# iclavera/learning_to_adapt

Hardware: AMD Instinct MI355X
Metric: controller-steps/sec (n_cand=2000, H=30, ens=5) (higher is better)
Workload: dtype f32

## Files before the change

### learning_to_adapt_amd/csrc/l2a_mfma.h

```cpp
#pragma once

#include <type_traits>

#include "l2a_kernels.h"

#ifndef L2A_XEARLY
#define L2A_XEARLY 1
#endif

#ifndef L2A_NW
#define L2A_NW 4
#endif

typedef unsigned int u32x4 __attribute__((ext_vector_type(4)));
__device__ __forceinline__ __amdgpu_buffer_rsrc_t l2a_rsrc(const void* base, long long bytes) {
    return __builtin_amdgcn_make_buffer_rsrc(const_cast<void*>(base), 0, (int)bytes, 0x00020000);
}
__device__ __forceinline__ f32x4 l2a_ldw(__amdgpu_buffer_rsrc_t rs, int voff, int soff) {
    return __builtin_bit_cast(f32x4, __builtin_amdgcn_raw_buffer_load_b128(rs, voff, soff, 0));
}

template <bool GACT>
__device__ __forceinline__ f32x4 l2a_actv(f32x4 v, int kind, float floor) {
    if (GACT) return l2a_act4(v, kind);
    v.x = l2a_max_nan(v.x, floor); v.y = l2a_max_nan(v.y, floor);
    v.z = l2a_max_nan(v.z, floor); v.w = l2a_max_nan(v.w, floor);
    return v;
}

__device__ __forceinline__ float l2a_sum_xor16(float x) {
    const unsigned int u = __float_as_uint(x);
    const auto r = __builtin_amdgcn_permlane16_swap(u, u, false, false);
    return __uint_as_float(r[0]) + __uint_as_float(r[1]);
}
__device__ __forceinline__ float l2a_sum_xor32(float x) {
    const unsigned int u = __float_as_uint(x);
    const auto r = __builtin_amdgcn_permlane32_swap(u, u, false, false);
    return __uint_as_float(r[0]) + __uint_as_float(r[1]);
}

#define L2A_MFMA4(a, b, c) __builtin_amdgcn_mfma_f32_4x4x1f32((a), (b), (c), 0, 0, 0)

#define L2A_OPAQUE(v) asm volatile("" : "+v"(v))

#ifndef L2A_TIMELINE
#define L2A_TS(slot)
#else
#define L2A_TS(slot)                                                                        \
    if (p.dbg && pairid == 0 && e < 8 && grp < 2) {                                         \
        unsigned long long ts_;                                                             \
        asm volatile("s_memtime %0\n\ts_waitcnt lgkmcnt(0)" : "=s"(ts_) : : "memory");       \
        if (lane == 0) p.dbg[(((long long)(grp * p.h + t) * 8 + e) * 8 + wave) * 16 + (slot)] = ts_; \
    }
#endif

#define L2A_STAGE_MFMA(CA, CB)                                                             \
    _Pragma("unroll") for (int ii = 0; ii < 4; ++ii)                                       \
        _Pragma("unroll") for (int nt = 0; nt < NT; ++nt)                                  \
            _Pragma("unroll") for (int tt = TW - 1; tt >= 0; --tt)    \
                acc[nt][tt] = L2A_MFMA(CA[tt][ii], CB[nt][ii], acc[nt][tt]);

#define L2A_STAGE(CA, CB, FA, FB, SOFF, IMM, GF)                                           \
    {                                                                                      \
        _Pragma("unroll") for (int tt = 0; tt < TW; ++tt)                                  \
            FA[tt] = l2a_ldw(rs, voff[tt] + (IMM), (SOFF));                                \
        _Pragma("unroll") for (int nt = 0; nt < NT; ++nt)                                  \
            FB[nt] = hin[(nt * HT + (GF)) * 64 + lane];                                    \
        L2A_STAGE_MFMA(CA, CB)                                                             \
         \
        __builtin_amdgcn_sched_group_barrier(0x100, NT, 0);                                \
        _Pragma("unroll") for (int tt = 0; tt < TW; ++tt) {                                \
            __builtin_amdgcn_sched_group_barrier(0x008, 4 * NT, 0);                        \
            __builtin_amdgcn_sched_group_barrier(0x020, 1, 0);                             \
        }                                                                                  \
        __builtin_amdgcn_sched_barrier(0);                                                 \
    }

#define L2A_PFT_MAX 6
#define L2A_PFT(TW_, OT_) ((OT_) <= 2 ? ((TW_) < L2A_PFT_MAX ? (TW_) : L2A_PFT_MAX) : ((TW_) < 2 ? (TW_) : 2))

template <int NT, int TW, int TPW, int OT, bool LAST>
__device__ __forceinline__ void l2a_hidden_gemm(__amdgpu_buffer_rsrc_t rs, __amdgpu_buffer_rsrc_t rsn,
                                                const int (&voff)[TPW], const int (&voffn)[TPW], int twn,
                                                int tile0, const f32x4* hin,
                                                f32x4 (&aA)[TPW], f32x4 (&aB)[TPW],
                                                f32x4 (&pfO)[TPW][OT], f32x4 (&acc)[NT][TPW], int lane,
                                                const float* bias_lds, f32x4 (&bias)[TPW], const int (&olane)[OT]) {
    constexpr int HT = L2A_NW * TPW;
    static_assert(HT % 4 == 0, "the k-group pipeline is unrolled by 4");
    f32x4 aC[TW], aD[TW], bA[NT], bB[NT], bC[NT], bD[NT];
#pragma unroll
    for (int nt = 0; nt < NT; ++nt) {
        bA[nt] = hin[(nt * HT + 0) * 64 + lane];
        bB[nt] = hin[(nt * HT + 1) * 64 + lane];
#pragma unroll
        for (int tt = 0; tt < TW; ++tt) acc[nt][tt] = (f32x4){0.f, 0.f, 0.f, 0.f};
    }
#pragma unroll
    for (int nt = 0; nt < NT; ++nt) { L2A_OPAQUE(bA[nt]); L2A_OPAQUE(bB[nt]); }
    __builtin_amdgcn_sched_barrier(0);

#pragma unroll 1
    for (int g = 0; g < HT - 4; g += 4) {
        const int soff = (g + 2) * 1024;
        L2A_STAGE(aA, bA, aC, bC, soff, 0, g + 2)
        L2A_STAGE(aB, bB, aD, bD, soff, 1024, g + 3)
        L2A_STAGE(aC, bC, aA, bA, soff, 2048, g + 4)
        L2A_STAGE(aD, bD, aB, bB, soff, 3072, g + 5)
    }
    L2A_STAGE(aA, bA, aC, bC, (HT - 2) * 1024, 0, HT - 2)
    L2A_STAGE(aB, bB, aD, bD, (HT - 2) * 1024, 1024, HT - 1)
    {
        if (LAST) {
#pragma unroll
            for (int tt = 0; tt < L2A_PFT(TW, OT); ++tt)
#pragma unroll
                for (int c = 0; c < OT; ++c)
                    if (((tt * OT + c) & 1) == 0)
                        pfO[tt][c] = l2a_ldw(rsn, olane[c] + (tile0 + tt) * 1024, c * HT * 1024);
        } else {
#pragma unroll
            for (int tt = 0; tt < TPW; ++tt)
                if (tt < twn) aA[tt] = l2a_ldw(rsn, voffn[tt], 0);
        }
        L2A_STAGE_MFMA(aC, bC)
        __builtin_amdgcn_sched_barrier(0);
    }
    {
#pragma unroll
        for (int tt = 0; tt < TW; ++tt) bias[tt] = *reinterpret_cast<const f32x4*>(bias_lds + 16 * tt);
        if (LAST) {
#pragma unroll
            for (int tt = 0; tt < L2A_PFT(TW, OT); ++tt)
#pragma unroll
                for (int c = 0; c < OT; ++c)
                    if (((tt * OT + c) & 1) == 1)
                        pfO[tt][c] = l2a_ldw(rsn, olane[c] + (tile0 + tt) * 1024, c * HT * 1024);
        } else {
#pragma unroll
            for (int tt = 0; tt < TPW; ++tt)
                if (tt < twn) aB[tt] = l2a_ldw(rsn, voffn[tt] + 1024, 0);
        }
        L2A_STAGE_MFMA(aD, bD)
        __builtin_amdgcn_sched_barrier(0);
    }
}

template <int NT, int TW, int TPW, int OT, int NPF, bool O4, class PF>
__device__ __forceinline__ void l2a_out_phase(const f32x4 (&hreg)[NT][TPW], f32x4 (&pfO)[TPW][OT],
                                              __amdgpu_buffer_rsrc_t rs_out, int tile0, PF prefetch,
                                              f32x4* pbuf, int chunk0, int lane, const int (&olane)[OT]) {
    constexpr int HT = L2A_NW * TPW;
    constexpr int CS = TPW / 2;
    constexpr int NCH = TW / CS;
    f32x4 a[TW][OT];
#pragma unroll
    for (int tt = 0; tt < TW; ++tt)
#pragma unroll
        for (int c = 0; c < OT; ++c)
            a[tt][c] = (tt < L2A_PFT(TW, OT)) ? pfO[tt][c]
                                              : l2a_ldw(rs_out, olane[c] + (tile0 + tt) * 1024, c * HT * 1024);
    prefetch();
    f32x4 acc[NCH][NT][OT];
#pragma unroll
    for (int ch = 0; ch < NCH; ++ch)
#pragma unroll
        for (int nt = 0; nt < NT; ++nt)
#pragma unroll
            for (int c = 0; c < OT; ++c) acc[ch][nt][c] = (f32x4){0.f, 0.f, 0.f, 0.f};
#pragma unroll
    for (int t2 = 0; t2 < CS; ++t2)
#pragma unroll
        for (int ii = 0; ii < 4; ++ii)
#pragma unroll
            for (int ch = 0; ch < NCH; ++ch)
#pragma unroll
                for (int nt = 0; nt < NT; ++nt)
#pragma unroll
                    for (int c = 0; c < OT; ++c)
                        acc[ch][nt][c] = (O4 && c == OT - 1)
                            ? L2A_MFMA4(a[ch * CS + t2][c][ii], hreg[nt][ch * CS + t2][ii], acc[ch][nt][c])
                            : L2A_MFMA(a[ch * CS + t2][c][ii], hreg[nt][ch * CS + t2][ii], acc[ch][nt][c]);
    {
        constexpr int NLATE = (TW - L2A_PFT(TW, OT)) * OT;
        constexpr int NMFMA = TW * 4 * NT * OT;
#pragma unroll
        for (int i = 0; i < NLATE; ++i) {
            __builtin_amdgcn_sched_group_barrier(0x020, 1, 0);
            __builtin_amdgcn_sched_group_barrier(0x008, 2, 0);
        }
        constexpr int PER = (NMFMA - 2 * NLATE) / NPF > 0 ? (NMFMA - 2 * NLATE) / NPF : 1;
#pragma unroll
        for (int i = 0; i < NPF; ++i) {
            __builtin_amdgcn_sched_group_barrier(0x008, PER, 0);
            __builtin_amdgcn_sched_group_barrier(0x020, 1, 0);
        }
    }
#pragma unroll
    for (int nt = 0; nt < NT; ++nt)
#pragma unroll
        for (int c = 0; c < OT; ++c)
            pbuf[((chunk0 * NT + nt) * OT + c) * 64 + lane] = (NCH == 2) ? acc[0][nt][c] + acc[NCH - 1][nt][c] : acc[0][nt][c];
}

template <int NT, int TPW, int OT, int KG0, bool GACT, int K0L = 4, bool N1 = false, bool O4 = false, bool FAN = false, bool WHOLE = false>
__global__ void __launch_bounds__(64 * L2A_NW) l2a_rollout_mfma_k(const L2AKParams p) {
    static_assert(!(FAN && WHOLE), "an instance is general, member fan or whole-tiles-only");
    constexpr bool NOHALF = FAN || WHOLE;
    constexpr int HT = L2A_NW * TPW;
    constexpr int TH = TPW / 2;
    static_assert(TPW % 2 == 0, "half members split a wave's tiles in two");
    constexpr int CST_BOUT = 32 * KG0 + 32 * OT;
    constexpr int CST_BHID = CST_BOUT + 16 * OT;
    constexpr int PS = L2A_NW * NT * OT * 64;
    const int NRM_SET = p.cst_set;
    const int LB = p.lb;
    extern __shared__ __attribute__((aligned(16))) char l2a_smem[];
    f32x4* buf0 = reinterpret_cast<f32x4*>(l2a_smem);
    f32x4* buf1 = buf0 + p.sa_elems;
    f32x4* pbase = buf0 + (LB > 1 ? LB : 2) * p.sa_elems;
    float* nrm = reinterpret_cast<float*>(buf0 + p.cst_off);

    const int tid = threadIdx.x;
    const int lane = tid & 63;
    const int wave = __builtin_amdgcn_readfirstlane(tid >> 6);
    const int jc = lane & 15;
    const int qq = lane >> 4;
    const int c0 = wave * TPW;
    int olane[OT];
#pragma unroll
    for (int c = 0; c < OT; ++c) olane[c] = ((O4 && c == OT - 1) ? ((lane & 48) | (lane & 3)) : lane) * 16;

    const int tail = p.split_from >= 0;
    const int in_tail = tail && (int)blockIdx.x >= p.split_from;
    const int split = FAN ? 3 : WHOLE ? 0 : (tail ? (in_tail ? p.split : 0) : p.split);
    const int n_tiles = p.m * p.tiles_per_env;
    const int n_pairs = tail ? n_tiles - p.split_from : n_tiles;
    int bid, grp, lpair, pairid;
    if (!tail && p.pl_units > 0) {
        const int hx = (int)blockIdx.x & 7, idx = (int)blockIdx.x >> 3;
        const int xcd = hx;
        const int f = p.pl_f, wide = p.pl_r * (f + 1);
        int u, k, xu;
        if (xcd < wide) { u = xcd / (f + 1); k = xcd - u * (f + 1); xu = f + 1; }
        else { const int y = xcd - wide; u = y / f; k = y - u * f; u += p.pl_r; xu = f; }
        const int su = (p.pl_w + xu - 1) / xu;
        const int j = k * su + idx;
        if (idx >= su || j >= p.pl_w) return;
        if (p.mode == L2A_MODE_PER_BLOCK) {
            grp = split ? j / p.tiles_per_env : 0;
            lpair = u * p.tiles_per_env + (j - grp * p.tiles_per_env);
        } else {
            grp = u;
            lpair = j;
        }
        bid = grp * n_pairs + lpair;
        pairid = lpair;
    } else if (!tail) {
        bid = l2a_logical_wg(blockIdx.x, gridDim.x);
        grp = split ? (bid / n_pairs) : 0;
        lpair = bid - grp * n_pairs;
        pairid = lpair;
    } else if (!in_tail) {
        bid = l2a_logical_wg(blockIdx.x, p.split_from);
        grp = 0; lpair = 0; pairid = bid;
    } else {
        bid = (int)blockIdx.x - p.split_from;
        grp = bid & 1; lpair = bid >> 1;
        pairid = p.split_from + lpair;
    }
#if defined(L2A_TIMELINE) || defined(L2A_WGREC)
    unsigned long long wg_t0_, wg_r0_;
    asm volatile("s_memtime %0\n\ts_memrealtime %1\n\ts_waitcnt lgkmcnt(0)" : "=s"(wg_t0_), "=s"(wg_r0_) : : "memory");
#endif
    const int env = pairid / p.tiles_per_env;
    const int tb = pairid - env * p.tiles_per_env;
    const int R = p.m * p.n;
    const int obs_dim = p.obs_dim, act_dim = p.act_dim;
    const int n_hidden = N1 ? 1 : p.n_hidden;

    int cand[NT], row[NT];
    bool valid[NT];
#pragma unroll
    for (int nt = 0; nt < NT; ++nt) {
        cand[nt] = p.c_lo + tb * (16 * NT) + nt * 16 + jc;
        valid[nt] = cand[nt] < p.c_hi;
        row[nt] = env * p.n + (valid[nt] ? cand[nt] : p.c_hi - 1);
    }

    const bool per_block = (p.mode == L2A_MODE_PER_BLOCK);
    const int e_loop = (p.mode == L2A_MODE_MEAN) ? p.n_sets : 1;
    const int e_half = (e_loop + 1) >> 1;
    const int e_shared = (!NOHALF && split == 2) ? e_half - 1 : -1;
    const int n_full = FAN ? 1 : (!split ? e_loop : (grp == 0 ? e_half - (split == 2 ? 1 : 0) : e_loop - e_half));
    const int n_seq = FAN ? 1 : n_full + (split == 2 ? 1 : 0);
    const int full0 = FAN ? grp : ((split && grp == 1) ? e_half : 0);
    auto seq = [&](int i) { return (i < n_full) ? full0 + i : e_shared; };
    auto set_base = [&](int e) { return p.wblk + (long long)(per_block ? env : e) * p.set_stride; };

    f32x4* xlds = reinterpret_cast<f32x4*>(nrm + p.n_cst * NRM_SET);
    for (int i = tid; i < n_seq * NRM_SET; i += 64 * L2A_NW) {
        const int s = i / NRM_SET;
        const int o = i - s * NRM_SET;
        const float* src = set_base(seq(s));
        float v;
        if (o < CST_BOUT) v = src[p.nm_off + o];
        else if (o < CST_BHID) v = src[p.pk_bout + (o - CST_BOUT)];
        else {
            const int l = (o - CST_BHID) / (16 * HT);
            v = src[p.raw_b[l] + (o - CST_BHID - l * 16 * HT)];
        }
        nrm[i] = v;
    }

    f32x4 st[NT][OT];
#pragma unroll
    for (int nt = 0; nt < NT; ++nt) {
        const float* orow = p.obs0 + (p.obs_per_row ? (long long)row[nt] : (long long)env) * obs_dim;
#pragma unroll
        for (int c = 0; c < OT; ++c)
#pragma unroll
            for (int ii = 0; ii < 4; ++ii) {
                const int dim = 16 * c + 4 * qq + ii;
                const float v = orow[dim < obs_dim ? dim : obs_dim - 1];
                st[nt][c][ii] = (dim < obs_dim) ? v : 0.0f;
            }
    }
    __syncthreads();

    const int ga0 = obs_dim >> 4;
    f32x4 av_next[NT][2];
    int aoff[NT][2][4];
#pragma unroll
    for (int nt = 0; nt < NT; ++nt)
#pragma unroll
        for (int s = 0; s < 2; ++s)
#pragma unroll
            for (int ii = 0; ii < 4; ++ii) {
                const int ka = 16 * (ga0 + s) + 4 * qq + ii - obs_dim;
                const bool in = (ka >= 0) && (ka < act_dim);
                aoff[nt][s][ii] = in ? (row[nt] * act_dim + ka) * 4 : 0x7ffffff0;
            }
    const long long a_step = (long long)R * act_dim;
    auto load_actions = [&](int t, f32x4 (&dst)[NT][2]) {
        const __amdgpu_buffer_rsrc_t ars = l2a_rsrc(p.actions + (long long)t * a_step, a_step * 4);
#pragma unroll
        for (int nt = 0; nt < NT; ++nt)
#pragma unroll
            for (int s = 0; s < 2; ++s)
#pragma unroll
                for (int ii = 0; ii < 4; ++ii)
                    dst[nt][s][ii] = __builtin_bit_cast(float, __builtin_amdgcn_raw_buffer_load_b32(ars, aoff[nt][s][ii], 0, 0));
    };
    f32x4 av[NT][2];
    float asq[NT];
    auto take_actions = [&](int t_fetch) {
#pragma unroll
        for (int nt = 0; nt < NT; ++nt) {
            av[nt][0] = av_next[nt][0];
            av[nt][1] = av_next[nt][1];
            float s = 0.0f;
#pragma unroll
            for (int ii = 0; ii < 4; ++ii) {
                s = fmaf(av[nt][0][ii], av[nt][0][ii], s);
                s = fmaf(av[nt][1][ii], av[nt][1][ii], s);
            }
            asq[nt] = s;
        }
        load_actions((t_fetch < p.h) ? t_fetch : p.h - 1, av_next);
    };
    load_actions(0, av_next);
    take_actions(1);

    float ret[NT];
#pragma unroll
    for (int nt = 0; nt < NT; ++nt) ret[nt] = p.ret_in ? p.ret_in[(long long)env * p.n + (valid[nt] ? cand[nt] : p.c_hi - 1)] : 0.0f;

    f32x4* hcur = buf0;
    f32x4* hoth = buf1;
    const float e_count = (float)e_loop;
    const float e_inv = 1.0f / e_count;
    double disc_pow = p.disc0;
    unsigned int spin_left = p.spin_limit;
    const unsigned int xtag0 = p.xtag;
    const __amdgpu_buffer_rsrc_t xrs = l2a_rsrc(p.xbuf, FAN ? (long long)n_pairs * e_loop * 2 * (NT * OT * 2 * 64 * 16)
                                                        : split ? (long long)n_pairs * 8 * (NT * OT * 2 * 64 * 16) : 16);

    constexpr int KG0P = (FAN && KG0 <= 2) ? KG0 : 1;
    f32x4 pfL0[KG0P][TPW];
    f32x4 pfA[TPW], pfB[TPW];
    f32x4 pfO[TPW][OT];
    int voff[TPW], voffh[TPW], voff0[TPW];
    const int tile0h = grp * (HT / 2) + wave * TH;
#pragma unroll
    for (int tt = 0; tt < TPW; ++tt) {
        voff[tt] = lane * 16 + (c0 + tt) * HT * 1024;
        voffh[tt] = lane * 16 + (tile0h + (tt < TH ? tt : 0)) * HT * 1024;
        voff0[tt] = lane * 16 + (c0 + tt) * KG0 * 1024;
    }
    const long long w0_bytes = (long long)HT * KG0 * 1024, wm_bytes = (long long)HT * HT * 1024,
                    wo_bytes = (long long)OT * HT * 1024;
    {
        const __amdgpu_buffer_rsrc_t r0 = l2a_rsrc(set_base(seq(0)) + p.pk_w0, w0_bytes);
#pragma unroll
        for (int g = 0; g < KG0P; ++g)
#pragma unroll
            for (int tt = 0; tt < TPW; ++tt) pfL0[g][tt] = l2a_ldw(r0, voff0[tt] + g * 1024, 0);
    }

    for (int t = 0; t < p.h; ++t) {
        f32x4 dsum[NT][OT], dgrp[NT][OT], qsh[NT][OT];
#pragma unroll
        for (int nt = 0; nt < NT; ++nt)
#pragma unroll
            for (int c = 0; c < OT; ++c) {
                dsum[nt][c] = (f32x4){0.f, 0.f, 0.f, 0.f};
                dgrp[nt][c] = (f32x4){0.f, 0.f, 0.f, 0.f};
                qsh[nt][c] = (f32x4){0.f, 0.f, 0.f, 0.f};
            }

        const unsigned int xtag = xtag0 + (unsigned int)(t + 1);
        constexpr int XREG = NT * OT * 2 * 64 * 16;
        auto xbase = [&](int g, int region) { return (((lpair * 2 + g) * 2 + (t & 1)) * 2 + region) * XREG + lane * 16; };
        auto xput = [&](int region, const f32x4 (&v)[NT][OT]) {
#pragma unroll
            for (int nt = 0; nt < NT; ++nt)
#pragma unroll
                for (int c = 0; c < OT; ++c)
#pragma unroll
                    for (int hh = 0; hh < 2; ++hh) {
                        u32x4 g;
                        g.x = xtag; g.y = __float_as_uint(v[nt][c][2 * hh]);
                        g.z = xtag; g.w = __float_as_uint(v[nt][c][2 * hh + 1]);
                        __builtin_amdgcn_raw_buffer_store_b128(g, xrs, xbase(grp, region) + ((nt * OT + c) * 2 + hh) * 1024, 0, L2A_SC1);
                    }
        };
        auto xget = [&](int region, f32x4 (&v)[NT][OT]) {
            bool ok = true;
#pragma unroll
            for (int nt = 0; nt < NT; ++nt)
#pragma unroll
                for (int c = 0; c < OT; ++c)
#pragma unroll
                    for (int hh = 0; hh < 2; ++hh) {
                        const u32x4 g = __builtin_amdgcn_raw_buffer_load_b128(
                            xrs, xbase(grp ^ 1, region) + ((nt * OT + c) * 2 + hh) * 1024, 0, L2A_SC1);
                        v[nt][c][2 * hh] = __uint_as_float(g.y);
                        v[nt][c][2 * hh + 1] = __uint_as_float(g.w);
                        ok = ok && (g.x == xtag) && (g.z == xtag);
                    }
            return ok;
        };

        bool xearly = false;
        u32x4 sw[2][NT][OT][2];
        for (int b0 = 0; b0 < n_seq; b0 += LB) {
            const int nb = (n_seq - b0 < LB) ? n_seq - b0 : LB;
            f32x4 hreg[NT][TPW];

            auto layer0 = [&](int j, auto last_tag) {
                constexpr bool last_l0 = decltype(last_tag)::value;
                const int i = b0 + j;
                const int e = seq(i);
                const float* wb = set_base(e);
                const float* nr = nrm + i * NRM_SET;
                const __amdgpu_buffer_rsrc_t rs_out = l2a_rsrc(wb + p.pk_wout, wo_bytes);
                L2A_TS(0)
                const __amdgpu_buffer_rsrc_t r0 = l2a_rsrc(wb + p.pk_w0, w0_bytes);
                f32x4 a[KG0][TPW];
#pragma unroll
                for (int g = 0; g < KG0; ++g)
#pragma unroll
                    for (int tt = 0; tt < TPW; ++tt)
                        a[g][tt] = (g < KG0P) ? pfL0[g < KG0P ? g : 0][tt] : l2a_ldw(r0, voff0[tt] + g * 1024, 0);
                L2A_TS(8)
                constexpr bool XPRE = (KG0 <= 2);
                auto norm_in = [&](int g, const f32x4& mu, const f32x4& iv, f32x4 (&x)[NT]) {
#pragma unroll
                    for (int nt = 0; nt < NT; ++nt) {
                        f32x4 sv = (f32x4){0.f, 0.f, 0.f, 0.f};
                        if (g < OT) sv = st[nt][g < OT ? g : 0];
                        f32x4 aa = (f32x4){0.f, 0.f, 0.f, 0.f};
                        if (g == ga0) aa = av[nt][0];
                        if (g == ga0 + 1) aa = av[nt][1];
#pragma unroll
                        for (int ii = 0; ii < 4; ++ii) x[nt][ii] = ((sv[ii] + aa[ii]) - mu[ii]) * iv[ii];
                    }
                };
                f32x4 xin[XPRE ? KG0 : 1][NT];
                if (XPRE) {
                    f32x4 mu[KG0], iv[KG0];
#pragma unroll
                    for (int g = 0; g < KG0; ++g) {
                        mu[g] = *reinterpret_cast<const f32x4*>(nr + 16 * g + 4 * qq);
                        iv[g] = *reinterpret_cast<const f32x4*>(nr + 16 * KG0 + 16 * g + 4 * qq);
                    }
                    __builtin_amdgcn_sched_barrier(0);
#pragma unroll
                    for (int g = 0; g < KG0; ++g) norm_in(g, mu[g], iv[g], xin[XPRE ? g : 0]);
                }
                f32x4 bias0[TPW];
#pragma unroll
                for (int tt = 0; tt < TPW; ++tt)
                    bias0[tt] = *reinterpret_cast<const f32x4*>(nr + CST_BHID + 16 * (c0 + tt) + 4 * qq);
                f32x4 acc[NT][TPW];
                auto l0_mfma = [&](auto npf_tag) {
                    constexpr int NPF = decltype(npf_tag)::value;
#pragma unroll
                    for (int nt = 0; nt < NT; ++nt)
#pragma unroll
                        for (int tt = 0; tt < TPW; ++tt) acc[nt][tt] = (f32x4){0.f, 0.f, 0.f, 0.f};
#pragma unroll
                    for (int g = 0; g < KG0; ++g) {
                        f32x4 xg[NT];
                        if (XPRE) {
#pragma unroll
                            for (int nt = 0; nt < NT; ++nt) xg[nt] = xin[XPRE ? g : 0][nt];
                        } else {
                            const f32x4 mu = *reinterpret_cast<const f32x4*>(nr + 16 * g + 4 * qq);
                            const f32x4 iv = *reinterpret_cast<const f32x4*>(nr + 16 * KG0 + 16 * g + 4 * qq);
                            norm_in(g, mu, iv, xg);
                        }
#pragma unroll
                        for (int ii = 0; ii < 4; ++ii) {
                            if (g == KG0 - 1 && ii >= K0L) continue;
#pragma unroll
                            for (int nt = 0; nt < NT; ++nt)
#pragma unroll
                                for (int tt = 0; tt < TPW; ++tt)
                                    acc[nt][tt] = L2A_MFMA(a[g][tt][ii], xg[nt][ii], acc[nt][tt]);
                        }
                    }
                    constexpr int NM = ((KG0 - 1) * 4 + K0L) * NT * TPW;
                    constexpr int PER = NM / (NPF > 0 ? NPF : 1) > 0 ? NM / (NPF > 0 ? NPF : 1) : 1;
                    __builtin_amdgcn_sched_group_barrier(0x020, (KG0 - KG0P) * TPW, 0);
#pragma unroll
                    for (int k = 0; k < NPF; ++k) {
                        __builtin_amdgcn_sched_group_barrier(0x008, PER, 0);
                        __builtin_amdgcn_sched_group_barrier(0x020, 1, 0);
                    }
                };
                if (N1) {
#pragma unroll
                    for (int tt = 0; tt < L2A_PFT(TPW, OT); ++tt)
#pragma unroll
                        for (int c = 0; c < OT; ++c)
                            pfO[tt][c] = l2a_ldw(rs_out, olane[c] + (c0 + tt) * 1024, c * HT * 1024);
                    l0_mfma(std::integral_constant<int, L2A_PFT(TPW, OT) * OT>{});
                } else if (!last_l0) {
                    const __amdgpu_buffer_rsrc_t r0n = l2a_rsrc(set_base(seq(i + 1)) + p.pk_w0, w0_bytes);
#pragma unroll
                    for (int g = 0; g < KG0P; ++g)
#pragma unroll
                        for (int tt = 0; tt < TPW; ++tt) pfL0[g][tt] = l2a_ldw(r0n, voff0[tt] + g * 1024, 0);
                    l0_mfma(std::integral_constant<int, KG0P * TPW>{});
                } else {
                    const int e0 = seq(b0);
                    const __amdgpu_buffer_rsrc_t rs1 = l2a_rsrc(set_base(e0) + p.pk_wmid, wm_bytes);
                    const bool next_half = !NOHALF && (e0 == e_shared) && n_hidden == 2;
                    if (next_half) {
#pragma unroll
                        for (int tt = 0; tt < TH; ++tt) {
                            pfA[tt] = l2a_ldw(rs1, voffh[tt], 0);
                            pfB[tt] = l2a_ldw(rs1, voffh[tt] + 1024, 0);
                        }
                        l0_mfma(std::integral_constant<int, 2 * TH>{});
                    } else {
#pragma unroll
                        for (int tt = 0; tt < TPW; ++tt) {
                            pfA[tt] = l2a_ldw(rs1, voff[tt], 0);
                            pfB[tt] = l2a_ldw(rs1, voff[tt] + 1024, 0);
                        }
                        l0_mfma(std::integral_constant<int, 2 * TPW>{});
                    }
                }
                L2A_TS(9)
#pragma unroll
                for (int tt = 0; tt < TPW; ++tt) {
#pragma unroll
                    for (int nt = 0; nt < NT; ++nt)
                        hreg[nt][tt] = l2a_actv<GACT>(acc[nt][tt] + bias0[tt], p.hidden_act, p.hid_floor);
                }
                L2A_TS(10)
                if (!N1) {
                    f32x4* hdst = (LB > 1) ? buf0 + j * p.sa_elems : hcur;
#pragma unroll
                    for (int tt = 0; tt < TPW; ++tt)
#pragma unroll
                        for (int nt = 0; nt < NT; ++nt) hdst[(nt * HT + c0 + tt) * 64 + lane] = hreg[nt][tt];
                }
                L2A_TS(1)
            };

            auto member = [&](int j, auto last_tag) {
                constexpr bool last_set = decltype(last_tag)::value;
                const int i = b0 + j;
                const int e = seq(i);
                const bool is_half = !NOHALF && last_set && (e == e_shared);
                const float* wb = set_base(e);
                const float* nr = nrm + i * NRM_SET;
                const __amdgpu_buffer_rsrc_t rs_out = l2a_rsrc(wb + p.pk_wout, wo_bytes);
                f32x4* pb = (LB > 1) ? pbase + j * PS : hoth;
                L2A_TS(2)
                if (!N1) {
                    f32x4 acc[NT][TPW], bias[TPW];
                    for (int l = 1; last_set && l < n_hidden - 1; ++l) {
                        const float* wl = wb + p.pk_wmid + (long long)(l - 1) * p.pk_wmid_stride;
                        const bool next_half = is_half && (l == n_hidden - 2);
                        l2a_hidden_gemm<NT, TPW, TPW, OT, false>(l2a_rsrc(wl, wm_bytes), l2a_rsrc(wl + p.pk_wmid_stride, wm_bytes),
                                                                 voff, next_half ? voffh : voff, next_half ? TH : TPW, 0,
                                                                 hcur, pfA, pfB, pfO, acc, lane,
                                                                 nr + CST_BHID + l * (16 * HT) + 16 * c0 + 4 * qq, bias, olane);
#pragma unroll
                        for (int tt = 0; tt < TPW; ++tt) {
#pragma unroll
                            for (int nt = 0; nt < NT; ++nt)
                                hoth[(nt * HT + c0 + tt) * 64 + lane] = l2a_actv<GACT>(acc[nt][tt] + bias[tt], p.hidden_act, p.hid_floor);
                        }
                        __syncthreads();
                        f32x4* tmp = hcur; hcur = hoth; hoth = tmp;
                    }
                    if (LB == 1) pb = hoth;
                    L2A_TS(15)
                    const f32x4* hin = (LB > 1) ? buf0 + j * p.sa_elems : hcur;
                    const __amdgpu_buffer_rsrc_t rs_last =
                        l2a_rsrc(wb + p.pk_wmid + (long long)(n_hidden - 2) * p.pk_wmid_stride, wm_bytes);
                    const float* bl = nr + CST_BHID + (n_hidden - 1) * (16 * HT);
                    if (!is_half) {
                        l2a_hidden_gemm<NT, TPW, TPW, OT, true>(rs_last, rs_out, voff, voff, TPW, c0, hin, pfA, pfB, pfO,
                                                                acc, lane, bl + 16 * c0 + 4 * qq, bias, olane);
#pragma unroll
                        for (int tt = 0; tt < TPW; ++tt) {
#pragma unroll
                            for (int nt = 0; nt < NT; ++nt)
                                hreg[nt][tt] = l2a_actv<GACT>(acc[nt][tt] + bias[tt], p.hidden_act, p.hid_floor);
                        }
                    } else {
                        l2a_hidden_gemm<NT, TH, TPW, OT, true>(rs_last, rs_out, voffh, voffh, TH, tile0h, hin, pfA, pfB,
                                                               pfO, acc, lane, bl + 16 * tile0h + 4 * qq, bias, olane);
#pragma unroll
                        for (int tt = 0; tt < TH; ++tt) {
#pragma unroll
                            for (int nt = 0; nt < NT; ++nt)
                                hreg[nt][tt] = l2a_actv<GACT>(acc[nt][tt] + bias[tt], p.hidden_act, p.hid_floor);
                        }
                    }
                }
                L2A_TS(3)
                if (last_set) {
                    const __amdgpu_buffer_rsrc_t r0n = l2a_rsrc(set_base(seq((i + 1 < n_seq) ? i + 1 : 0)) + p.pk_w0, w0_bytes);
                    auto pf_l0 = [&]() {
#pragma unroll
                        for (int g = 0; g < KG0P; ++g)
#pragma unroll
                            for (int tt = 0; tt < TPW; ++tt) pfL0[g][tt] = l2a_ldw(r0n, voff0[tt] + g * 1024, 0);
                    };
                    if (is_half) l2a_out_phase<NT, TH, TPW, OT, KG0P * TPW, O4>(hreg, pfO, rs_out, tile0h, pf_l0, pb, wave, lane, olane);
                    else l2a_out_phase<NT, TPW, TPW, OT, KG0P * TPW, O4>(hreg, pfO, rs_out, c0, pf_l0, pb, wave, lane, olane);
                } else {
                    const int en = seq(i + 1);
                    const __amdgpu_buffer_rsrc_t rsn = l2a_rsrc(set_base(en) + p.pk_wmid, wm_bytes);
                    if (!NOHALF && en == e_shared) {
                        l2a_out_phase<NT, TPW, TPW, OT, 2 * TH, O4>(hreg, pfO, rs_out, c0, [&]() {
#pragma unroll
                            for (int tt = 0; tt < TH; ++tt) {
                                pfA[tt] = l2a_ldw(rsn, voffh[tt], 0);
                                pfB[tt] = l2a_ldw(rsn, voffh[tt] + 1024, 0);
                            }
                        }, pb, wave, lane, olane);
                    } else {
                        l2a_out_phase<NT, TPW, TPW, OT, 2 * TPW, O4>(hreg, pfO, rs_out, c0, [&]() {
#pragma unroll
                            for (int tt = 0; tt < TPW; ++tt) {
                                pfA[tt] = l2a_ldw(rsn, voff[tt], 0);
                                pfB[tt] = l2a_ldw(rsn, voff[tt] + 1024, 0);
                            }
                        }, pb, wave, lane, olane);
                    }
                }
                L2A_TS(4)
            };
            for (int j = 0; j + 1 < nb; ++j) layer0(j, std::false_type{});
            layer0(nb - 1, std::true_type{});
            if (!N1) __syncthreads();
            for (int j = 0; j + 1 < nb; ++j) member(j, std::false_type{});
            member(nb - 1, std::true_type{});

            __syncthreads();
            constexpr bool XE_OK = L2A_XEARLY && !NOHALF && NT == 1 && OT <= 2 && KG0 <= 2;
            const bool xe = XE_OK && split == 2 && nb >= 2 && b0 + nb == n_seq;
            for (int jj = 0; jj < nb; ++jj) {
                const int j = (xe && wave == 0) ? (jj == 0 ? nb - 1 : jj - 1) : jj;
                const int i = b0 + j;
                const int e = seq(i);
                const bool is_half = !NOHALF && (e == e_shared);
                const float* nr = nrm + i * NRM_SET;
                const f32x4* pb = (LB > 1) ? pbase + j * PS : hoth;
                L2A_TS(5)
                if (e == e_half && !split) {
#pragma unroll
                    for (int nt = 0; nt < NT; ++nt)
#pragma unroll
                        for (int c = 0; c < OT; ++c) {
                            dsum[nt][c] = dgrp[nt][c];
                            dgrp[nt][c] = (f32x4){0.f, 0.f, 0.f, 0.f};
                        }
                }
#pragma unroll
                for (int c = 0; c < OT; ++c) {
                    f32x4 part[L2A_NW][NT];
#pragma unroll
                    for (int ch = 0; ch < L2A_NW; ++ch)
#pragma unroll
                        for (int nt = 0; nt < NT; ++nt) part[ch][nt] = pb[((ch * NT + nt) * OT + c) * 64 + lane];
                    const f32x4 bias = *reinterpret_cast<const f32x4*>(nr + CST_BOUT + 16 * c + 4 * qq);
                    const f32x4 omu = *reinterpret_cast<const f32x4*>(nr + 32 * KG0 + 16 * c + 4 * qq);
                    const f32x4 osd = *reinterpret_cast<const f32x4*>(nr + 32 * KG0 + 16 * OT + 16 * c + 4 * qq);
                    __builtin_amdgcn_sched_barrier(0);
#pragma unroll
                    for (int nt = 0; nt < NT; ++nt) {
                        static_assert(L2A_NW == 4, "the canonical tree below is written out for four waves");
                        f32x4 s = (part[0][nt] + part[1][nt]) + (part[2][nt] + part[3][nt]);
                        if (is_half) {
                            qsh[nt][c] = s;
                        } else {
                            if (O4 && c == OT - 1) {
#pragma unroll
                                for (int ii = 0; ii < 4; ++ii) s[ii] = l2a_sum_xor32(l2a_sum_xor16(s[ii]));
                            }
                            s = l2a_actv<GACT>(s + bias, p.output_act, p.out_floor);
                            if (FAN) dgrp[nt][c] = s * osd + omu;
                            else dgrp[nt][c] += s * osd + omu;
                        }
                    }
                }
                if (!NOHALF && split == 2 && i == n_full - 1 && wave == (XE_OK ? 1 : 0)) xput(0, dgrp);
                if (xe && wave == 0 && jj == 0) xput(1, qsh);
                if (xe && wave == 3 && jj == nb - 1) {
#pragma unroll
                    for (int r = 0; r < 2; ++r)
#pragma unroll
                        for (int nt = 0; nt < NT; ++nt)
#pragma unroll
                            for (int c = 0; c < OT; ++c)
#pragma unroll
                                for (int hh = 0; hh < 2; ++hh)
                                    sw[r][nt][c][hh] = (r == 1 || e_loop > 1)
                                        ? __builtin_amdgcn_raw_buffer_load_b128(xrs, xbase(grp ^ 1, r) + ((nt * OT + c) * 2 + hh) * 1024, 0, L2A_SC1)
                                        : (u32x4){xtag, 0u, xtag, 0u};
                }
                L2A_TS(6)
            }
            if (xe) xearly = true;
            if (N1) { f32x4* tmp = hcur; hcur = hoth; hoth = tmp; }
        }

        { const int e = 7; L2A_TS(9) }
        float asq_t[NT];
#pragma unroll
        for (int nt = 0; nt < NT; ++nt) asq_t[nt] = asq[nt];
        if (FAN) {
            constexpr int XREGF = NT * OT * 2 * 64 * 16;
            auto fbase = [&](int g) { return ((lpair * e_loop + g) * 2 + (t & 1)) * XREGF + lane * 16; };
            if (wave == 0) {
#pragma unroll
                for (int nt = 0; nt < NT; ++nt)
#pragma unroll
                    for (int c = 0; c < OT; ++c) {
#pragma unroll
                        for (int hh = 0; hh < 2; ++hh) {
                            u32x4 g;
                            g.x = xtag; g.y = __float_as_uint(dgrp[nt][c][2 * hh]);
                            g.z = xtag; g.w = __float_as_uint(dgrp[nt][c][2 * hh + 1]);
                            __builtin_amdgcn_raw_buffer_store_b128(g, xrs, fbase(grp) + ((nt * OT + c) * 2 + hh) * 1024, 0, L2A_SC1);
                        }
                        xlds[((grp * NT + nt) * OT + c) * 64 + lane] = dgrp[nt][c];
                    }
            }
            { const int e = 7; L2A_TS(11) }
            take_actions(t + 2);
            for (int k = wave; k < e_loop - 1; k += L2A_NW) {
                int g2 = grp + 1 + k;
                if (g2 >= e_loop) g2 -= e_loop;
                f32x4 oth[NT][OT];
                while (true) {
                    bool ok = true;
#pragma unroll
                    for (int nt = 0; nt < NT; ++nt)
#pragma unroll
                        for (int c = 0; c < OT; ++c)
#pragma unroll
                            for (int hh = 0; hh < 2; ++hh) {
                                const u32x4 g = __builtin_amdgcn_raw_buffer_load_b128(
                                    xrs, fbase(g2) + ((nt * OT + c) * 2 + hh) * 1024, 0, L2A_SC1);
                                oth[nt][c][2 * hh] = __uint_as_float(g.y);
                                oth[nt][c][2 * hh + 1] = __uint_as_float(g.w);
                                ok = ok && (g.x == xtag) && (g.z == xtag);
                            }
                    if (__all(ok)) break;
                    if (spin_left == 0) {
                        if (lane == 0) __hip_atomic_fetch_or(p.status, 1u, __ATOMIC_RELAXED, __HIP_MEMORY_SCOPE_SYSTEM);
                        break;
                    }
                    --spin_left;
                    __builtin_amdgcn_s_sleep(4);
                }
#pragma unroll
                for (int nt = 0; nt < NT; ++nt)
#pragma unroll
                    for (int c = 0; c < OT; ++c) xlds[((g2 * NT + nt) * OT + c) * 64 + lane] = oth[nt][c];
            }
            { const int e = 7; L2A_TS(12) }
            __syncthreads();
            { const int e = 7; L2A_TS(13) }
#pragma unroll
            for (int nt = 0; nt < NT; ++nt)
#pragma unroll
                for (int c = 0; c < OT; ++c) {
                    dsum[nt][c] = (f32x4){0.f, 0.f, 0.f, 0.f};
                    dgrp[nt][c] = (f32x4){0.f, 0.f, 0.f, 0.f};
                }
            {
                constexpr int EMAX = 8;
                f32x4 v[EMAX][NT][OT];
#pragma unroll
                for (int e = 0; e < EMAX; ++e) {
                    const int es = e < e_loop ? e : e_loop - 1;
#pragma unroll
                    for (int nt = 0; nt < NT; ++nt)
#pragma unroll
                        for (int c = 0; c < OT; ++c) v[e][nt][c] = xlds[((es * NT + nt) * OT + c) * 64 + lane];
                }
                __builtin_amdgcn_sched_barrier(0);
#pragma unroll
                for (int e = 0; e < EMAX; ++e)
#pragma unroll
                    for (int nt = 0; nt < NT; ++nt)
#pragma unroll
                        for (int c = 0; c < OT; ++c) {
                            if (e < e_half) dsum[nt][c] += v[e][nt][c];
                            else if (e < e_loop) dgrp[nt][c] += v[e][nt][c];
                        }
            }
        } else if (!WHOLE && split) {
            if (wave == 0 && !xearly) {
                if (split == 2) xput(1, qsh);
                else xput(0, dgrp);
            }
            { const int e = 7; L2A_TS(11) }
            take_actions(t + 2);
            if (xearly && wave == 3) {
                while (true) {
                    bool ok = true;
#pragma unroll
                    for (int r = 0; r < 2; ++r)
#pragma unroll
                        for (int nt = 0; nt < NT; ++nt)
#pragma unroll
                            for (int c = 0; c < OT; ++c)
#pragma unroll
                                for (int hh = 0; hh < 2; ++hh)
                                    ok = ok && (sw[r][nt][c][hh].x == xtag) && (sw[r][nt][c][hh].z == xtag);
                    if (__all(ok)) break;
                    if (spin_left == 0) {
                        if (lane == 0) __hip_atomic_fetch_or(p.status, 1u, __ATOMIC_RELAXED, __HIP_MEMORY_SCOPE_SYSTEM);
                        break;
                    }
                    --spin_left;
                    __builtin_amdgcn_s_sleep(4);
#pragma unroll
                    for (int r = 0; r < 2; ++r)
#pragma unroll
                        for (int nt = 0; nt < NT; ++nt)
#pragma unroll
                            for (int c = 0; c < OT; ++c)
#pragma unroll
                                for (int hh = 0; hh < 2; ++hh)
                                    if (r == 1 || e_loop > 1)
                                        sw[r][nt][c][hh] = __builtin_amdgcn_raw_buffer_load_b128(
                                            xrs, xbase(grp ^ 1, r) + ((nt * OT + c) * 2 + hh) * 1024, 0, L2A_SC1);
                }
#pragma unroll
                for (int r = 0; r < 2; ++r)
#pragma unroll
                    for (int nt = 0; nt < NT; ++nt)
#pragma unroll
                        for (int c = 0; c < OT; ++c) {
                            f32x4 v;
                            v[0] = __uint_as_float(sw[r][nt][c][0].y); v[1] = __uint_as_float(sw[r][nt][c][0].w);
                            v[2] = __uint_as_float(sw[r][nt][c][1].y); v[3] = __uint_as_float(sw[r][nt][c][1].w);
                            xlds[((r * NT + nt) * OT + c) * 64 + lane] = v;
// ... 175 lines not shown
```

Baseline: 703.3.

## Overlap previous member's output reduction with next member's last hidden GEMM

Moves the cross-wave output reduction for ensemble member j-1 into the last-hidden-layer GEMM of member j. The reduction's LDS reads and VALU adds are interleaved with the MFMA stages through scheduling group barriers, with an extra barrier placed after the first stage. After the final sync only the last member's reduction is left. Weight offsets are also changed from per-tile VGPR arrays to a scalar base plus stride, to lower register pressure. The risks are higher register use and a tighter, more fragile instruction schedule.

```diff
diff --git a/learning_to_adapt_amd/csrc/l2a_mfma.h b/learning_to_adapt_amd/csrc/l2a_mfma.h
--- a/learning_to_adapt_amd/csrc/l2a_mfma.h
+++ b/learning_to_adapt_amd/csrc/l2a_mfma.h
@@ -6,6 +6,13 @@
 
 #ifndef L2A_XEARLY
 #define L2A_XEARLY 1
+#endif
+
+#ifndef L2A_REDUCE_EARLY
+#define L2A_REDUCE_EARLY 1
+#endif
+#ifndef L2A_XREQ_SLEEP
+#define L2A_XREQ_SLEEP 0
 #endif
 
 #ifndef L2A_NW
@@ -18,6 +25,14 @@
 }
 __device__ __forceinline__ f32x4 l2a_ldw(__amdgpu_buffer_rsrc_t rs, int voff, int soff) {
     return __builtin_bit_cast(f32x4, __builtin_amdgcn_raw_buffer_load_b128(rs, voff, soff, 0));
+}
+struct L2AOff { int v, s, stride; };
+__device__ __forceinline__ f32x4 l2a_ldt(__amdgpu_buffer_rsrc_t rs, const L2AOff& o, int tt, int imm, int soff) {
+    return __builtin_bit_cast(f32x4, __builtin_amdgcn_raw_buffer_load_b128(rs, o.v + imm, soff + o.s + tt * o.stride, 0));
+}
+template <int N>
+__device__ __forceinline__ f32x4 l2a_ldt(__amdgpu_buffer_rsrc_t rs, const int (&voff)[N], int tt, int imm, int soff) {
+    return l2a_ldw(rs, voff[tt] + imm, soff);
 }
 
 template <bool GACT>
@@ -41,6 +56,14 @@
 
 #define L2A_MFMA4(a, b, c) __builtin_amdgcn_mfma_f32_4x4x1f32((a), (b), (c), 0, 0, 0)
 
+template <int N, int I = 0, class F>
+__device__ __forceinline__ void l2a_for_tiles(F&& f) {
+    if constexpr (I < N) {
+        f(std::integral_constant<int, I>{});
+        l2a_for_tiles<N, I + 1>(f);
+    }
+}
+
 #define L2A_OPAQUE(v) asm volatile("" : "+v"(v))
 
 #ifndef L2A_TIMELINE
@@ -63,7 +86,7 @@
 #define L2A_STAGE(CA, CB, FA, FB, SOFF, IMM, GF)                                           \
     {                                                                                      \
         _Pragma("unroll") for (int tt = 0; tt < TW; ++tt)                                  \
-            FA[tt] = l2a_ldw(rs, voff[tt] + (IMM), (SOFF));                                \
+            FA[tt] = l2a_ldt(rs, voff, tt, (IMM), (SOFF));                                \
         _Pragma("unroll") for (int nt = 0; nt < NT; ++nt)                                  \
             FB[nt] = hin[(nt * HT + (GF)) * 64 + lane];                                    \
         L2A_STAGE_MFMA(CA, CB)                                                             \
@@ -76,16 +99,35 @@
         __builtin_amdgcn_sched_barrier(0);                                                 \
     }
 
+#define L2A_STAGE_R(CA, CB, FA, FB, SOFF, IMM, GF, ND, NV)                                 \
+    {                                                                                      \
+        _Pragma("unroll") for (int tt = 0; tt < TW; ++tt)                                  \
+            FA[tt] = l2a_ldt(rs, voff, tt, (IMM), (SOFF));                                \
+        _Pragma("unroll") for (int nt = 0; nt < NT; ++nt)                                  \
+            FB[nt] = hin[(nt * HT + (GF)) * 64 + lane];                                    \
+        L2A_STAGE_MFMA(CA, CB)                                                             \
+        __builtin_amdgcn_sched_group_barrier(0x100, NT + (ND), 0);                         \
+        _Pragma("unroll") for (int tt = 0; tt < TW; ++tt) {                                \
+            _Pragma("unroll") for (int mm = 0; mm < 4 * NT; ++mm) {                        \
+                __builtin_amdgcn_sched_group_barrier(0x008, 1, 0);                         \
+                __builtin_amdgcn_sched_group_barrier(0x002, (NV), 0);                      \
+            }                                                                              \
+            __builtin_amdgcn_sched_group_barrier(0x020, 1, 0);                             \
+        }                                                                                  \
+        __builtin_amdgcn_sched_barrier(0);                                                 \
+    }
+
 #define L2A_PFT_MAX 6
 #define L2A_PFT(TW_, OT_) ((OT_) <= 2 ? ((TW_) < L2A_PFT_MAX ? (TW_) : L2A_PFT_MAX) : ((TW_) < 2 ? (TW_) : 2))
 
-template <int NT, int TW, int TPW, int OT, bool LAST>
+template <int NT, int TW, int TPW, int OT, bool LAST, bool RED = false, class RED_F = int>
 __device__ __forceinline__ void l2a_hidden_gemm(__amdgpu_buffer_rsrc_t rs, __amdgpu_buffer_rsrc_t rsn,
-                                                const int (&voff)[TPW], const int (&voffn)[TPW], int twn,
+                                                const L2AOff voff, const L2AOff voffn, int twn,
                                                 int tile0, const f32x4* hin,
                                                 f32x4 (&aA)[TPW], f32x4 (&aB)[TPW],
                                                 f32x4 (&pfO)[TPW][OT], f32x4 (&acc)[NT][TPW], int lane,
-                                                const float* bias_lds, f32x4 (&bias)[TPW], const int (&olane)[OT]) {
+                                                const float* bias_lds, f32x4 (&bias)[TPW], const int (&olane)[OT],
+                                                RED_F red = RED_F()) {
     constexpr int HT = L2A_NW * TPW;
     static_assert(HT % 4 == 0, "the k-group pipeline is unrolled by 4");
     f32x4 aC[TW], aD[TW], bA[NT], bB[NT], bC[NT], bD[NT];
@@ -100,8 +142,21 @@
     for (int nt = 0; nt < NT; ++nt) { L2A_OPAQUE(bA[nt]); L2A_OPAQUE(bB[nt]); }
     __builtin_amdgcn_sched_barrier(0);
 
+    if constexpr (RED) {
+        red(std::integral_constant<int, 0>{});
+        L2A_STAGE(aA, bA, aC, bC, 2 * 1024, 0, 2)
+        asm volatile("s_waitcnt lgkmcnt(0)\n\ts_barrier" ::: "memory");
+        __builtin_amdgcn_sched_barrier(0);
+        red(std::integral_constant<int, 1>{});
+        L2A_STAGE_R(aB, bB, aD, bD, 2 * 1024, 1024, 3, OT * (L2A_NW * NT + 3), 0)
+        L2A_STAGE(aC, bC, aA, bA, 2 * 1024, 2048, 4)
+        red(std::integral_constant<int, 2>{});
+        red(std::integral_constant<int, 3>{});
+        L2A_STAGE_R(aD, bD, aB, bB, 2 * 1024, 3072, 5, 0, 3)
+        red(std::integral_constant<int, 4>{});
+    }
 #pragma unroll 1
-    for (int g = 0; g < HT - 4; g += 4) {
+    for (int g = RED ? 4 : 0; g < HT - 4; g += 4) {
         const int soff = (g + 2) * 1024;
         L2A_STAGE(aA, bA, aC, bC, soff, 0, g + 2)
         L2A_STAGE(aB, bB, aD, bD, soff, 1024, g + 3)
@@ -121,7 +176,7 @@
         } else {
 #pragma unroll
             for (int tt = 0; tt < TPW; ++tt)
-                if (tt < twn) aA[tt] = l2a_ldw(rsn, voffn[tt], 0);
+                if (tt < twn) aA[tt] = l2a_ldt(rsn, voffn, tt, 0, 0);
         }
         L2A_STAGE_MFMA(aC, bC)
         __builtin_amdgcn_sched_barrier(0);
@@ -139,7 +194,7 @@
         } else {
 #pragma unroll
             for (int tt = 0; tt < TPW; ++tt)
-                if (tt < twn) aB[tt] = l2a_ldw(rsn, voffn[tt] + 1024, 0);
+                if (tt < twn) aB[tt] = l2a_ldt(rsn, voffn, tt, 1024, 0);
         }
         L2A_STAGE_MFMA(aD, bD)
         __builtin_amdgcn_sched_barrier(0);
@@ -390,14 +445,9 @@
     f32x4 pfL0[KG0P][TPW];
     f32x4 pfA[TPW], pfB[TPW];
     f32x4 pfO[TPW][OT];
-    int voff[TPW], voffh[TPW], voff0[TPW];
-    const int tile0h = grp * (HT / 2) + wave * TH;
-#pragma unroll
-    for (int tt = 0; tt < TPW; ++tt) {
-        voff[tt] = lane * 16 + (c0 + tt) * HT * 1024;
-        voffh[tt] = lane * 16 + (tile0h + (tt < TH ? tt : 0)) * HT * 1024;
-        voff0[tt] = lane * 16 + (c0 + tt) * KG0 * 1024;
-    }
+    const int tile0h = __builtin_amdgcn_readfirstlane(grp * (HT / 2) + wave * TH);
+    const L2AOff voff = {lane * 16, c0 * HT * 1024, HT * 1024}, voffh = {lane * 16, tile0h * HT * 1024, HT * 1024},
+                 voff0 = {lane * 16, c0 * KG0 * 1024, KG0 * 1024};
     const long long w0_bytes = (long long)HT * KG0 * 1024, wm_bytes = (long long)HT * HT * 1024,
                     wo_bytes = (long long)OT * HT * 1024;
     {
@@ -405,7 +455,7 @@
 #pragma unroll
         for (int g = 0; g < KG0P; ++g)
 #pragma unroll
-            for (int tt = 0; tt < TPW; ++tt) pfL0[g][tt] = l2a_ldw(r0, voff0[tt] + g * 1024, 0);
+            for (int tt = 0; tt < TPW; ++tt) pfL0[g][tt] = l2a_ldt(r0, voff0, tt, g * 1024, 0);
     }
 
     for (int t = 0; t < p.h; ++t) {
@@ -472,7 +522,7 @@
                 for (int g = 0; g < KG0; ++g)
 #pragma unroll
                     for (int tt = 0; tt < TPW; ++tt)
-                        a[g][tt] = (g < KG0P) ? pfL0[g < KG0P ? g : 0][tt] : l2a_ldw(r0, voff0[tt] + g * 1024, 0);
+                        a[g][tt] = (g < KG0P) ? pfL0[g < KG0P ? g : 0][tt] : l2a_ldt(r0, voff0, tt, g * 1024, 0);
                 L2A_TS(8)
                 constexpr bool XPRE = (KG0 <= 2);
                 auto norm_in = [&](int g, const f32x4& mu, const f32x4& iv, f32x4 (&x)[NT]) {
@@ -552,7 +602,7 @@
 #pragma unroll
                     for (int g = 0; g < KG0P; ++g)
 #pragma unroll
-                        for (int tt = 0; tt < TPW; ++tt) pfL0[g][tt] = l2a_ldw(r0n, voff0[tt] + g * 1024, 0);
+                        for (int tt = 0; tt < TPW; ++tt) pfL0[g][tt] = l2a_ldt(r0n, voff0, tt, g * 1024, 0);
                     l0_mfma(std::integral_constant<int, KG0P * TPW>{});
                 } else {
                     const int e0 = seq(b0);
@@ -561,15 +611,15 @@
                     if (next_half) {
 #pragma unroll
                         for (int tt = 0; tt < TH; ++tt) {
-                            pfA[tt] = l2a_ldw(rs1, voffh[tt], 0);
-                            pfB[tt] = l2a_ldw(rs1, voffh[tt] + 1024, 0);
+                            pfA[tt] = l2a_ldt(rs1, voffh, tt, 0, 0);
+                            pfB[tt] = l2a_ldt(rs1, voffh, tt, 1024, 0);
                         }
                         l0_mfma(std::integral_constant<int, 2 * TH>{});
                     } else {
 #pragma unroll
                         for (int tt = 0; tt < TPW; ++tt) {
-                            pfA[tt] = l2a_ldw(rs1, voff[tt], 0);
-                            pfB[tt] = l2a_ldw(rs1, voff[tt] + 1024, 0);
+                            pfA[tt] = l2a_ldt(rs1, voff, tt, 0, 0);
+                            pfB[tt] = l2a_ldt(rs1, voff, tt, 1024, 0);
                         }
                         l0_mfma(std::integral_constant<int, 2 * TPW>{});
                     }
@@ -592,8 +642,54 @@
                 L2A_TS(1)
             };
 
-            auto member = [&](int j, auto last_tag) {
+            constexpr bool XE_OK = L2A_XEARLY && !NOHALF && NT == 1 && OT <= 2 && KG0 <= 2;
+            constexpr bool RE_OK = L2A_REDUCE_EARLY && !N1 && (NT == 1 || (NOHALF && OT <= 2));
+            auto red_park = [&](int i) {
+                if (seq(i) == e_half && !split) {
+#pragma unroll
+                    for (int nt = 0; nt < NT; ++nt)
+#pragma unroll
+                        for (int c = 0; c < OT; ++c) {
+                            dsum[nt][c] = dgrp[nt][c];
+                            dgrp[nt][c] = (f32x4){0.f, 0.f, 0.f, 0.f};
+                        }
+                }
+            };
+            auto red_read = [&](const f32x4* pb, const float* nr, int c, f32x4 (&part)[L2A_NW][NT], f32x4 (&k)[3]) {
+#pragma unroll
+                for (int ch = 0; ch < L2A_NW; ++ch)
+#pragma unroll
+                    for (int nt = 0; nt < NT; ++nt) part[ch][nt] = pb[((ch * NT + nt) * OT + c) * 64 + lane];
+                k[0] = *reinterpret_cast<const f32x4*>(nr + CST_BOUT + 16 * c + 4 * qq);
+                k[1] = *reinterpret_cast<const f32x4*>(nr + 32 * KG0 + 16 * c + 4 * qq);
+                k[2] = *reinterpret_cast<const f32x4*>(nr + 32 * KG0 + 16 * OT + 16 * c + 4 * qq);
+            };
+            auto red_add = [&](auto c_tag, const f32x4 (&part)[L2A_NW][NT], const f32x4 (&k)[3], bool is_half) {
+                constexpr int c = decltype(c_tag)::value;
+#pragma unroll
+                for (int nt = 0; nt < NT; ++nt) {
+                    static_assert(L2A_NW == 4, "the canonical tree below is written out for four waves");
+                    f32x4 s = (part[0][nt] + part[1][nt]) + (part[2][nt] + part[3][nt]);
+                    if (is_half) {
+                        qsh[nt][c] = s;
+                    } else {
+                        if (O4 && c == OT - 1) {
+#pragma unroll
+                            for (int ii = 0; ii < 4; ++ii) s[ii] = l2a_sum_xor32(l2a_sum_xor16(s[ii]));
+                        }
+                        s = l2a_actv<GACT>(s + k[0], p.output_act, p.out_floor);
+                        if (FAN) dgrp[nt][c] = s * k[2] + k[1];
+                        else dgrp[nt][c] += s * k[2] + k[1];
+                    }
+                }
+            };
+            auto red_publish = [&](int i) {
+                if (!NOHALF && split == 2 && i == n_full - 1 && wave == (XE_OK ? 1 : 0)) xput(0, dgrp);
+            };
+
+            auto member = [&](int j, auto last_tag, auto red_tag) {
                 constexpr bool last_set = decltype(last_tag)::value;
+                constexpr bool RED = decltype(red_tag)::value;
                 const int i = b0 + j;
                 const int e = seq(i);
                 const bool is_half = !NOHALF && last_set && (e == e_shared);
@@ -626,9 +722,30 @@
                     const __amdgpu_buffer_rsrc_t rs_last =
                         l2a_rsrc(wb + p.pk_wmid + (long long)(n_hidden - 2) * p.pk_wmid_stride, wm_bytes);
                     const float* bl = nr + CST_BHID + (n_hidden - 1) * (16 * HT);
+                    f32x4 rpart[RED ? OT : 1][L2A_NW][NT], rk[RED ? OT : 1][3];
+                    auto red = [&](auto step_tag) {
+                        constexpr int step = decltype(step_tag)::value;
+                        constexpr int CH = (OT + 1) / 2;
+                        if (step == 0) red_park(i - 1);
+#ifdef L2A_TIMELINE
+                        if (step == 1 || step == 4) { const int e = seq(i - 1); L2A_TS(step == 1 ? 5 : 6) }
+#endif
+                        if (step == 1) {
+#pragma unroll
+                            for (int c = 0; c < OT; ++c)
+                                red_read(pbase + (j - 1) * PS, nr - NRM_SET, c, rpart[RED ? c : 0], rk[RED ? c : 0]);
+                        }
+                        if (step == 2 || step == 3) {
+                            l2a_for_tiles<OT>([&](auto c_tag) {
+                                constexpr int c = decltype(c_tag)::value;
+                                if ((step == 2) == (c < CH)) red_add(c_tag, rpart[RED ? c : 0], rk[RED ? c : 0], false);
+                            });
+                        }
+                        if (step == 4) red_publish(i - 1);
+                    };
                     if (!is_half) {
-                        l2a_hidden_gemm<NT, TPW, TPW, OT, true>(rs_last, rs_out, voff, voff, TPW, c0, hin, pfA, pfB, pfO,
-                                                                acc, lane, bl + 16 * c0 + 4 * qq, bias, olane);
+                        l2a_hidden_gemm<NT, TPW, TPW, OT, true, RED>(rs_last, rs_out, voff, voff, TPW, c0, hin, pfA, pfB, pfO,
+                                                                     acc, lane, bl + 16 * c0 + 4 * qq, bias, olane, red);
 #pragma unroll
                         for (int tt = 0; tt < TPW; ++tt) {
 #pragma unroll
@@ -636,8 +753,8 @@
                                 hreg[nt][tt] = l2a_actv<GACT>(acc[nt][tt] + bias[tt], p.hidden_act, p.hid_floor);
                         }
                     } else {
-                        l2a_hidden_gemm<NT, TH, TPW, OT, true>(rs_last, rs_out, voffh, voffh, TH, tile0h, hin, pfA, pfB,
-                                                               pfO, acc, lane, bl + 16 * tile0h + 4 * qq, bias, olane);
+                        l2a_hidden_gemm<NT, TH, TPW, OT, true, RED>(rs_last, rs_out, voffh, voffh, TH, tile0h, hin, pfA, pfB,
+                                                                    pfO, acc, lane, bl + 16 * tile0h + 4 * qq, bias, olane, red);
 #pragma unroll
                         for (int tt = 0; tt < TH; ++tt) {
 #pragma unroll
@@ -653,7 +770,7 @@
 #pragma unroll
                         for (int g = 0; g < KG0P; ++g)
 #pragma unroll
-                            for (int tt = 0; tt < TPW; ++tt) pfL0[g][tt] = l2a_ldw(r0n, voff0[tt] + g * 1024, 0);
+                            for (int tt = 0; tt < TPW; ++tt) pfL0[g][tt] = l2a_ldt(r0n, voff0, tt, g * 1024, 0);
                     };
                     if (is_half) l2a_out_phase<NT, TH, TPW, OT, KG0P * TPW, O4>(hreg, pfO, rs_out, tile0h, pf_l0, pb, wave, lane, olane);
                     else l2a_out_phase<NT, TPW, TPW, OT, KG0P * TPW, O4>(hreg, pfO, rs_out, c0, pf_l0, pb, wave, lane, olane);
@@ -664,16 +781,16 @@
                         l2a_out_phase<NT, TPW, TPW, OT, 2 * TH, O4>(hreg, pfO, rs_out, c0, [&]() {
 #pragma unroll
                             for (int tt = 0; tt < TH; ++tt) {
-                                pfA[tt] = l2a_ldw(rsn, voffh[tt], 0);
-                                pfB[tt] = l2a_ldw(rsn, voffh[tt] + 1024, 0);
+                                pfA[tt] = l2a_ldt(rsn, voffh, tt, 0, 0);
+                                pfB[tt] = l2a_ldt(rsn, voffh, tt, 1024, 0);
                             }
                         }, pb, wave, lane, olane);
                     } else {
                         l2a_out_phase<NT, TPW, TPW, OT, 2 * TPW, O4>(hreg, pfO, rs_out, c0, [&]() {
 #pragma unroll
                             for (int tt = 0; tt < TPW; ++tt) {
-                                pfA[tt] = l2a_ldw(rsn, voff[tt], 0);
-                                pfB[tt] = l2a_ldw(rsn, voff[tt] + 1024, 0);
+                                pfA[tt] = l2a_ldt(rsn, voff, tt, 0, 0);
+                                pfB[tt] = l2a_ldt(rsn, voff, tt, 1024, 0);
                             }
                         }, pb, wave, lane, olane);
                     }
@@ -683,60 +800,41 @@
             for (int j = 0; j + 1 < nb; ++j) layer0(j, std::false_type{});
             layer0(nb - 1, std::true_type{});
             if (!N1) __syncthreads();
-            for (int j = 0; j + 1 < nb; ++j) member(j, std::false_type{});
-            member(nb - 1, std::true_type{});
+            if constexpr (RE_OK) {
+                if (nb > 1) {
+                    member(0, std::false_type{}, std::false_type{});
+                    for (int j = 1; j + 1 < nb; ++j) member(j, std::false_type{}, std::true_type{});
+                    member(nb - 1, std::true_type{}, std::true_type{});
+                } else {
+                    member(0, std::true_type{}, std::false_type{});
+                }
+            } else {
+                for (int j = 0; j + 1 < nb; ++j) member(j, std::false_type{}, std::false_type{});
+                member(nb - 1, std::true_type{}, std::false_type{});
+            }
 
             __syncthreads();
-            constexpr bool XE_OK = L2A_XEARLY && !NOHALF && NT == 1 && OT <= 2 && KG0 <= 2;
             const bool xe = XE_OK && split == 2 && nb >= 2 && b0 + nb == n_seq;
-            for (int jj = 0; jj < nb; ++jj) {
-                const int j = (xe && wave == 0) ? (jj == 0 ? nb - 1 : jj - 1) : jj;
+            const int jj0 = RE_OK ? nb - 1 : 0;
+            for (int jj = jj0; jj < nb; ++jj) {
+                const int j = RE_OK ? jj : (xe && wave == 0) ? (jj == 0 ? nb - 1 : jj - 1) : jj;
                 const int i = b0 + j;
                 const int e = seq(i);
                 const bool is_half = !NOHALF && (e == e_shared);
                 const float* nr = nrm + i * NRM_SET;
                 const f32x4* pb = (LB > 1) ? pbase + j * PS : hoth;
                 L2A_TS(5)
-                if (e == e_half && !split) {
-#pragma unroll
-                    for (int nt = 0; nt < NT; ++nt)
-#pragma unroll
-                        for (int c = 0; c < OT; ++c) {
-                            dsum[nt][c] = dgrp[nt][c];
-                            dgrp[nt][c] = (f32x4){0.f, 0.f, 0.f, 0.f};
-                        }
-                }
-#pragma unroll
-                for (int c = 0; c < OT; ++c) {
-                    f32x4 part[L2A_NW][NT];
-#pragma unroll
-                    for (int ch = 0; ch < L2A_NW; ++ch)
-#pragma unroll
-                        for (int nt = 0; nt < NT; ++nt) part[ch][nt] = pb[((ch * NT + nt) * OT + c) * 64 + lane];
-                    const f32x4 bias = *reinterpret_cast<const f32x4*>(nr + CST_BOUT + 16 * c + 4 * qq);
-                    const f32x4 omu = *reinterpret_cast<const f32x4*>(nr + 32 * KG0 + 16 * c + 4 * qq);
-                    const f32x4 osd = *reinterpret_cast<const f32x4*>(nr + 32 * KG0 + 16 * OT + 16 * c + 4 * qq);
+                red_park(i);
+                l2a_for_tiles<OT>([&](auto c_tag) {
+                    f32x4 part[L2A_NW][NT], k[3];
+                    red_read(pb, nr, decltype(c_tag)::value, part, k);
                     __builtin_amdgcn_sched_barrier(0);
-#pragma unroll
-                    for (int nt = 0; nt < NT; ++nt) {
-                        static_assert(L2A_NW == 4, "the canonical tree below is written out for four waves");
-                        f32x4 s = (part[0][nt] + part[1][nt]) + (part[2][nt] + part[3][nt]);
-                        if (is_half) {
-                            qsh[nt][c] = s;
-                        } else {
-                            if (O4 && c == OT - 1) {
-#pragma unroll
-                                for (int ii = 0; ii < 4; ++ii) s[ii] = l2a_sum_xor32(l2a_sum_xor16(s[ii]));
-                            }
-                            s = l2a_actv<GACT>(s + bias, p.output_act, p.out_floor);
-                            if (FAN) dgrp[nt][c] = s * osd + omu;
-                            else dgrp[nt][c] += s * osd + omu;
-                        }
-                    }
-                }
-                if (!NOHALF && split == 2 && i == n_full - 1 && wave == (XE_OK ? 1 : 0)) xput(0, dgrp);
-                if (xe && wave == 0 && jj == 0) xput(1, qsh);
+                    red_add(c_tag, part, k, is_half);
+                });
+                red_publish(i);
+                if (xe && wave == 0 && jj == jj0) xput(1, qsh);
                 if (xe && wave == 3 && jj == nb - 1) {
+                    if (RE_OK && L2A_XREQ_SLEEP > 0) __builtin_amdgcn_s_sleep(L2A_XREQ_SLEEP);
 #pragma unroll
                     for (int r = 0; r < 2; ++r)
 #pragma unroll
```

Result: slower. 694.6 (-1.2%).
